# TravisDai/DLRM-FlexFlow

Measured on AMD Instinct MI355X. Metric: samples/sec DLRM (MLPerf-like) at 1/2/4/8 MI355X; SOAP speedup vs pure DP, higher is better.
Workload: dtype fp32; 1 GPU; global_batch=8192, seq_len=1, parallelism=dp1, tables_rows=187767399, embedding_dim=128, interaction=dot, hip_graph=True, backend=none, process_world=1, fp32_gemm=bf16x3-split-big+native-f32-mfma, gemm_tuned_entries=21, gemm_staging=lds-dma

## Files before the change

csrc/kernels/embedding.hip:

```cpp
#include "common.h"

#include <algorithm>
#include <cstdlib>
#include <cstring>
#include <vector>

namespace {

constexpr int MAXT = 32;
constexpr int TINY_ROWS = 16;

struct TabDesc {
  const float* W;
  const void* idx;
  void* act;
  long ld;
  long lo;
  int rows, D, bag;
  float scale;
};

FM_DEVICE long local_row(long r, long lo, int rows, bool& ok) {
  const long l = r - lo;
  ok = (unsigned long)l < (unsigned long)rows;
  return ok ? l : 0;
}
struct TabSet {
  TabDesc t[MAXT];
  int n;
};

template <bool I64>
FM_DEVICE long ldi(const void* p, long i) {
  if constexpr (I64) return (long)reinterpret_cast<const long long*>(p)[i];
  else return (long)reinterpret_cast<const int*>(p)[i];
}

template <typename OutT, bool I64>
__global__ void __launch_bounds__(256) fm_emb_fwd_multi(TabSet s, long B, int su) {
  const TabDesc& d = s.t[blockIdx.y];
  const int D4 = d.D >> 2;
  const int lpr = D4 < 64 ? D4 : 64;
  const int rpi = 256 / lpr;
  const int sub = threadIdx.x / lpr, lc = threadIdx.x - sub * lpr;
  if (sub >= rpi) return;
  const long bstride = (long)gridDim.x * rpi;
  if (su && d.bag == 1 && D4 <= 64) {
    constexpr int SU = 4;
    const int c = lc * 4;
    for (long b0 = (long)blockIdx.x * rpi + sub; b0 < B; b0 += SU * bstride) {
      long r[SU];
      bool ok[SU];
#pragma unroll
      for (int u = 0; u < SU; ++u) r[u] = local_row(ldi<I64>(d.idx, min(b0 + u * bstride, B - 1)), d.lo, d.rows, ok[u]);
      f32x4_t v[SU];
#pragma unroll
      for (int u = 0; u < SU; ++u) v[u] = *reinterpret_cast<const f32x4_t*>(d.W + r[u] * d.D + c);
#pragma unroll
      for (int u = 0; u < SU; ++u) {
        const long b = b0 + u * bstride;
        if (b >= B) break;
        f32x4_t acc = ok[u] ? v[u] * d.scale : f32x4_t{0.f, 0.f, 0.f, 0.f};
        OutT* o = reinterpret_cast<OutT*>(d.act) + b * d.ld + c;
        if constexpr (sizeof(OutT) == 4) {
          *reinterpret_cast<f32x4_t*>(o) = acc;
        } else {
          bf16x4_t w;
          w[0] = (short)f2bf(acc[0]); w[1] = (short)f2bf(acc[1]); w[2] = (short)f2bf(acc[2]); w[3] = (short)f2bf(acc[3]);
          *reinterpret_cast<bf16x4_t*>(o) = w;
        }
      }
    }
    return;
  }
  for (long b = (long)blockIdx.x * rpi + sub; b < B; b += bstride) {
    for (int c4 = lc; c4 < D4; c4 += lpr) {
      const int c = c4 * 4;
      f32x4_t acc = {0.f, 0.f, 0.f, 0.f};
      int j = 0;
      for (; j + 8 <= d.bag; j += 8) {
        long r[8];
        bool ok[8];
#pragma unroll
        for (int u = 0; u < 8; ++u) r[u] = local_row(ldi<I64>(d.idx, b * d.bag + j + u), d.lo, d.rows, ok[u]);
        f32x4_t v[8];
#pragma unroll
        for (int u = 0; u < 8; ++u) v[u] = *reinterpret_cast<const f32x4_t*>(d.W + r[u] * d.D + c);
#pragma unroll
        for (int u = 0; u < 8; ++u)
          if (ok[u]) acc += v[u];
      }
      for (; j < d.bag; ++j) {
        bool ok;
        const long r = local_row(ldi<I64>(d.idx, b * d.bag + j), d.lo, d.rows, ok);
        const f32x4_t v = *reinterpret_cast<const f32x4_t*>(d.W + r * d.D + c);
        if (ok) acc += v;
      }
      acc *= d.scale;
      OutT* o = reinterpret_cast<OutT*>(d.act) + b * d.ld + c;
      if constexpr (sizeof(OutT) == 4) {
        *reinterpret_cast<f32x4_t*>(o) = acc;
      } else {
        bf16x4_t v;
        v[0] = (short)f2bf(acc[0]); v[1] = (short)f2bf(acc[1]); v[2] = (short)f2bf(acc[2]); v[3] = (short)f2bf(acc[3]);
        *reinterpret_cast<bf16x4_t*>(o) = v;
      }
    }
  }
}

template <typename OutT, bool I64>
__global__ void __launch_bounds__(256) fm_emb_fwd_split(TabSet s, long B, int sp) {
  __shared__ f32x4_t part[256];
  const TabDesc& d = s.t[blockIdx.y];
  const int lpr = d.D >> 2;
  const int rpi = 256 / lpr;
  const int spb = rpi / sp;
  const int sub = threadIdx.x / lpr, lc = threadIdx.x - sub * lpr;
  const bool live = sub < spb * sp;
  const int si = sub / sp, k = sub - si * sp;
  const long b = (long)blockIdx.x * spb + si;
  f32x4_t acc = {0.f, 0.f, 0.f, 0.f};
  if (live && b < B) {
    const int c = lc * 4;
    int j = k;
    for (; j + 3 * sp < d.bag; j += 4 * sp) {
      long r[4];
      bool ok[4];
#pragma unroll
      for (int u = 0; u < 4; ++u) r[u] = local_row(ldi<I64>(d.idx, b * d.bag + j + u * sp), d.lo, d.rows, ok[u]);
      f32x4_t v[4];
#pragma unroll
      for (int u = 0; u < 4; ++u) v[u] = *reinterpret_cast<const f32x4_t*>(d.W + r[u] * d.D + c);
#pragma unroll
      for (int u = 0; u < 4; ++u)
        if (ok[u]) acc += v[u];
    }
    for (; j < d.bag; j += sp) {
      bool ok;
      const long r = local_row(ldi<I64>(d.idx, b * d.bag + j), d.lo, d.rows, ok);
      const f32x4_t v = *reinterpret_cast<const f32x4_t*>(d.W + r * d.D + c);
      if (ok) acc += v;
    }
  }
  part[threadIdx.x] = acc;
  __syncthreads();
  if (!live || k != 0 || b >= B) return;
  for (int q = 1; q < sp; ++q) acc += part[threadIdx.x + q * lpr];
  acc *= d.scale;
  OutT* o = reinterpret_cast<OutT*>(d.act) + b * d.ld + lc * 4;
  if constexpr (sizeof(OutT) == 4) {
    *reinterpret_cast<f32x4_t*>(o) = acc;
  } else {
    bf16x4_t v;
    v[0] = (short)f2bf(acc[0]); v[1] = (short)f2bf(acc[1]); v[2] = (short)f2bf(acc[2]); v[3] = (short)f2bf(acc[3]);
    *reinterpret_cast<bf16x4_t*>(o) = v;
  }
}

template <typename OutT, bool I64>
__global__ void __launch_bounds__(256) fm_emb_fwd_multi_scalar(TabSet s, long B) {
  const TabDesc& d = s.t[blockIdx.y];
  const int lpr = d.D < 256 ? d.D : 256;
  const int rpi = 256 / lpr;
  const int sub = threadIdx.x / lpr, lc = threadIdx.x - sub * lpr;
  if (sub >= rpi) return;
  for (long b = (long)blockIdx.x * rpi + sub; b < B; b += (long)gridDim.x * rpi)
    for (int c = lc; c < d.D; c += lpr) {
      float acc = 0.f;
      for (int j = 0; j < d.bag; ++j) {
        bool ok;
        const long r = local_row(ldi<I64>(d.idx, b * d.bag + j), d.lo, d.rows, ok);
        const float v = d.W[r * d.D + c];
        if (ok) acc += v;
      }
      st<OutT>(reinterpret_cast<OutT*>(d.act) + b * d.ld + c, acc * d.scale);
    }
}

template <typename GT, bool I64>
__global__ void __launch_bounds__(256) fm_emb_bwd_atomic_multi(TabSet s, const float* __restrict__ lr, long B) {
  const TabDesc& d = s.t[blockIdx.y];
  const float mul = (lr ? -lr[0] : 1.f) * d.scale;
  const int lpr = d.D < 256 ? d.D : 256;
  const int rpi = 256 / lpr;
  const int sub = threadIdx.x / lpr, lc = threadIdx.x - sub * lpr;
  if (sub >= rpi) return;
  float* W = const_cast<float*>(d.W);
  const GT* dy = reinterpret_cast<const GT*>(d.act);
  for (long b = (long)blockIdx.x * rpi + sub; b < B; b += (long)gridDim.x * rpi) {
    bool ok0;
    const long r0 = local_row(ldi<I64>(d.idx, b * d.bag), d.lo, d.rows, ok0);
    for (int c = lc; c < d.D; c += lpr) {
      const float g = ld<GT>(dy + b * d.ld + c) * mul;
      if (ok0) atomicAdd(W + r0 * d.D + c, g);
      for (int j = 1; j < d.bag; ++j) {
        bool ok;
        const long r = local_row(ldi<I64>(d.idx, b * d.bag + j), d.lo, d.rows, ok);
        if (ok) atomicAdd(W + r * d.D + c, g);
      }
    }
  }
}

template <typename GT, bool I64>
__global__ void __launch_bounds__(256) fm_emb_bwd_tiny_multi(TabSet s, const float* __restrict__ lr, long B, int chunk) {
  constexpr int S = 16;
  extern __shared__ __attribute__((aligned(16))) char smem[];
  float* red = reinterpret_cast<float*>(smem);
  const TabDesc& d = s.t[blockIdx.y];
  const long b0 = (long)blockIdx.x * chunk;
  if (b0 >= B) return;
  const long b1 = min(B, b0 + chunk);
  const int wave = threadIdx.x >> 6, lane = threadIdx.x & 63;
  const int n = d.rows * d.D;
  float* mine = red + wave * n;
  for (int i = lane; i < n; i += 64) mine[i] = 0.f;
  const GT* dy = reinterpret_cast<const GT*>(d.act);
  for (long bw = b0 + (long)wave * S; bw < b1; bw += 4L * S) {
    for (int c0 = 0; c0 < d.D; c0 += 128) {
      const int ca = c0 + lane, cb = c0 + 64 + lane;
      const int sa = min(ca, d.D - 1), sb = min(cb, d.D - 1);
      long r[S];
      bool rok[S];
      float ga[S], gb[S];
#pragma unroll
      for (int u = 0; u < S; ++u) {
        const long bu = min(bw + u, b1 - 1);
        r[u] = local_row(ldi<I64>(d.idx, bu * d.bag), d.lo, d.rows, rok[u]);
        ga[u] = ld<GT>(dy + bu * d.ld + sa);
        gb[u] = ld<GT>(dy + bu * d.ld + sb);
      }
#pragma unroll
      for (int u = 0; u < S; ++u) {
        if (bw + u >= b1) break;
        float* p = mine + r[u] * d.D;
        if (rok[u] && ca < d.D) p[ca] += ga[u];
        if (rok[u] && cb < d.D) p[cb] += gb[u];
        for (int j = 1; j < d.bag; ++j) {
          bool ok;
          float* q = mine + local_row(ldi<I64>(d.idx, (bw + u) * d.bag + j), d.lo, d.rows, ok) * d.D;
          if (ok && ca < d.D) q[ca] += ga[u];
          if (ok && cb < d.D) q[cb] += gb[u];
        }
      }
    }
  }
  __syncthreads();
  const float mul = (lr ? -lr[0] : 1.f) * d.scale;
  float* W = const_cast<float*>(d.W);
  for (int i = threadIdx.x; i < n; i += 256) {
    const float v = red[i] + red[n + i] + red[2 * n + i] + red[3 * n + i];
    if (v != 0.f) atomicAdd(W + i, v * mul);
  }
}

template <bool I64>
void launch_fwd(const TabSet& s, int m, bool vec, bool out_bf16, long B, int D0, hipStream_t st) {
  const int rpi = std::max(1, 256 / std::min(64, std::max(1, D0 / 4)));
  int minbag = 1 << 30, maxD = 0, minD = 1 << 30;
  for (int i = 0; i < m; ++i) {
    minbag = std::min(minbag, s.t[i].bag);
    maxD = std::max(maxD, s.t[i].D);
    minD = std::min(minD, s.t[i].D);
  }
  if (vec && maxD == minD && maxD <= 256 && minbag >= 16 && (B + rpi - 1) / rpi * m < 1024) {
    int sp = 1;
    while (sp * 2 <= rpi && sp * 2 <= minbag / 4 && (B * sp * 2 + rpi - 1) / rpi * m <= 2048) sp *= 2;
    if (sp > 1) {
      const int spb = rpi / sp;
      dim3 grid((unsigned)((B + spb - 1) / spb), m);
      if (out_bf16) hipLaunchKernelGGL((fm_emb_fwd_split<unsigned short, I64>), grid, dim3(256), 0, st, s, B, sp);
      else hipLaunchKernelGGL((fm_emb_fwd_split<float, I64>), grid, dim3(256), 0, st, s, B, sp);
      return;
    }
  }
  dim3 grid((unsigned)std::max<long>(1, std::min<long>((B + rpi - 1) / rpi, 256L)), m);
  const int su = 1;
  if (vec) {
    if (out_bf16) hipLaunchKernelGGL((fm_emb_fwd_multi<unsigned short, I64>), grid, dim3(256), 0, st, s, B, su);
    else hipLaunchKernelGGL((fm_emb_fwd_multi<float, I64>), grid, dim3(256), 0, st, s, B, su);
  } else {
    if (out_bf16) hipLaunchKernelGGL((fm_emb_fwd_multi_scalar<unsigned short, I64>), grid, dim3(256), 0, st, s, B);
    else hipLaunchKernelGGL((fm_emb_fwd_multi_scalar<float, I64>), grid, dim3(256), 0, st, s, B);
  }
}

struct ClaimDesc {
  float* W;
  const void* idx;
  const void* dy;
  long ld;
  long lo;
  int rows, D, bag;
  float scale;
  int* owner;
  int* dups;
  int* ndup;
};
struct ClaimSet {
  ClaimDesc t[MAXT];
  int n;
};

template <bool I64>
__global__ void __launch_bounds__(256) fm_emb_claim_multi(ClaimSet s, long B) {
  const ClaimDesc& d = s.t[blockIdx.y];
  const long n = B * d.bag;
  for (long e = blockIdx.x * 256L + threadIdx.x; e < n; e += (long)gridDim.x * 256) {
    bool ok;
    const long r = local_row(ldi<I64>(d.idx, e), d.lo, d.rows, ok);
    if (!ok) continue;
    const int prev = atomicCAS(d.owner + r, -1, (int)e);
    if (prev != -1) d.dups[atomicAdd(d.ndup, 1)] = (int)e;
  }
}

template <typename GT, bool I64>
__global__ void __launch_bounds__(256) fm_emb_dup_multi(ClaimSet s, const float* __restrict__ lr) {
  const ClaimDesc& d = s.t[blockIdx.y];
  const int nd = *d.ndup;
  const float mul = -lr[0] * d.scale;
  const int wave = threadIdx.x >> 6, lane = threadIdx.x & 63;
  const GT* dy = reinterpret_cast<const GT*>(d.dy);
  for (long k = blockIdx.x * 4L + wave; k < nd; k += (long)gridDim.x * 4) {
    const long e = d.dups[k];
    const long b = e / d.bag, r = ldi<I64>(d.idx, e) - d.lo;
    for (int c = lane; c < d.D; c += 64) atomicAdd(d.W + r * d.D + c, ld<GT>(dy + b * d.ld + c) * mul);
  }
}

template <typename GT, bool I64>
__global__ void __launch_bounds__(256) fm_emb_owner_multi(ClaimSet s, const float* __restrict__ lr, long B) {
  const ClaimDesc& d = s.t[blockIdx.y];
  const float mul = -lr[0] * d.scale;
  const int D4 = d.D >> 2;
  const int lpr = D4 < 64 ? D4 : 64;
  const int rpi = 256 / lpr;
  const int sub = threadIdx.x / lpr, lc = threadIdx.x - sub * lpr;
  const long n = B * d.bag;
  const GT* dy = reinterpret_cast<const GT*>(d.dy);
  if (sub < rpi) {
    for (long e = (long)blockIdx.x * rpi + sub; e < n; e += (long)gridDim.x * rpi) {
      bool ok;
      const long r = local_row(ldi<I64>(d.idx, e), d.lo, d.rows, ok);
      if (!ok || d.owner[r] != (int)e) continue;
      const long b = e / d.bag;
      for (int c4 = lc; c4 < D4; c4 += lpr) {
        const int c = c4 * 4;
        f32x4_t* wp = reinterpret_cast<f32x4_t*>(d.W + r * d.D + c);
        f32x4_t w = *wp;
        if constexpr (sizeof(GT) == 2) {
          const bf16x4_t g = *reinterpret_cast<const bf16x4_t*>(dy + b * d.ld + c);
#pragma unroll
          for (int j = 0; j < 4; ++j) w[j] += mul * bf2f((unsigned short)g[j]);
        } else {
          const f32x4_t g = *reinterpret_cast<const f32x4_t*>(dy + b * d.ld + c);
          w += mul * g;
        }
        *wp = w;
      }
      if (lc == 0) d.owner[r] = -1;
    }
  }
  if (blockIdx.x == 0 && threadIdx.x == 0) *d.ndup = 0;
}

template <bool I64>
__global__ void __launch_bounds__(256) fm_emb_count_multi(ClaimSet s, long B) {
  const ClaimDesc& d = s.t[blockIdx.y];
  const long n = B * d.bag;
  for (long e = blockIdx.x * 256L + threadIdx.x; e < n; e += (long)gridDim.x * 256) {
    bool ok;
    const long r = local_row(ldi<I64>(d.idx, e), d.lo, d.rows, ok);
    int own = 0;
    if (ok) own = atomicAdd(d.owner + r, 1) == -1;
    d.dups[e] = own;
  }
}

template <typename GT, bool I64>
__global__ void __launch_bounds__(256) fm_emb_update_multi(ClaimSet s, const float* __restrict__ lr, long B) {
  const ClaimDesc& d = s.t[blockIdx.y];
  const float mul = -lr[0] * d.scale;
  const int D4 = d.D >> 2;
  const int lpr = D4 < 64 ? D4 : 64;
  const int rpi = 256 / lpr;
  const int sub = threadIdx.x / lpr, lc = threadIdx.x - sub * lpr;
  const long n = B * d.bag;
  const GT* dy = reinterpret_cast<const GT*>(d.dy);
  if (sub >= rpi) return;
  for (long e = (long)blockIdx.x * rpi + sub; e < n; e += (long)gridDim.x * rpi) {
    bool ok;
    const long r = local_row(ldi<I64>(d.idx, e), d.lo, d.rows, ok);
    if (!ok) continue;
    const int c = __hip_atomic_load(d.owner + r, __ATOMIC_RELAXED, __HIP_MEMORY_SCOPE_AGENT);
    const int own = d.dups[e];
    const long b = e / d.bag;
    const GT* g = dy + b * d.ld;
    float* wr = d.W + r * d.D;
    if (c == 0) {
      for (int c4 = lc; c4 < D4; c4 += lpr) {
        const int col = c4 * 4;
        f32x4_t* wp = reinterpret_cast<f32x4_t*>(wr + col);
        f32x4_t w = *wp;
        if constexpr (sizeof(GT) == 2) {
          const bf16x4_t gv = *reinterpret_cast<const bf16x4_t*>(g + col);
#pragma unroll
          for (int j = 0; j < 4; ++j) w[j] += mul * bf2f((unsigned short)gv[j]);
        } else {
          w += mul * *reinterpret_cast<const f32x4_t*>(g + col);
        }
        *wp = w;
      }
    } else {
      for (int col = lc; col < d.D; col += lpr) atomicAdd(wr + col, mul * ld<GT>(g + col));
    }
    if (lc == 0 && (c == 0 || own)) __hip_atomic_store(d.owner + r, -1, __ATOMIC_RELAXED, __HIP_MEMORY_SCOPE_AGENT);
  }
}

template <bool I64>
void launch_count(const ClaimSet& s, int m, bool dy_bf16, const float* lr, long B, int maxbag, int minD4,
                  hipStream_t st) {
  const long n = B * maxbag;
  dim3 gc((unsigned)std::max<long>(1, std::min<long>((n + 255) / 256, 1024)), m);
  hipLaunchKernelGGL((fm_emb_count_multi<I64>), gc, dim3(256), 0, st, s, B);
  const int rpi = 256 / std::min(64, std::max(1, minD4));
  dim3 gu((unsigned)std::max<long>(1, std::min<long>((n + rpi - 1) / rpi, 2048)), m);
  if (dy_bf16) hipLaunchKernelGGL((fm_emb_update_multi<unsigned short, I64>), gu, dim3(256), 0, st, s, lr, B);
  else hipLaunchKernelGGL((fm_emb_update_multi<float, I64>), gu, dim3(256), 0, st, s, lr, B);
}

long emb_bwd_cap(long want) { return want; }

template <bool I64>
void launch_claim(const ClaimSet& s, int m, bool dy_bf16, const float* lr, long B, int maxbag, int minD4,
                  hipStream_t st) {
  const long n = B * maxbag;
  dim3 gc((unsigned)std::max<long>(1, emb_bwd_cap(std::min<long>((n + 255) / 256, 1024))), m);
  hipLaunchKernelGGL((fm_emb_claim_multi<I64>), gc, dim3(256), 0, st, s, B);
  dim3 gd((unsigned)std::max<long>(1, emb_bwd_cap(std::min<long>((n + 3) / 4, 1024))), m);
  if (dy_bf16) hipLaunchKernelGGL((fm_emb_dup_multi<unsigned short, I64>), gd, dim3(256), 0, st, s, lr);
  else hipLaunchKernelGGL((fm_emb_dup_multi<float, I64>), gd, dim3(256), 0, st, s, lr);
  const int rpi = 256 / std::min(64, std::max(1, minD4));
  dim3 go((unsigned)std::max<long>(1, emb_bwd_cap(std::min<long>((n + rpi - 1) / rpi, 2048))), m);
  if (dy_bf16) hipLaunchKernelGGL((fm_emb_owner_multi<unsigned short, I64>), go, dim3(256), 0, st, s, lr, B);
  else hipLaunchKernelGGL((fm_emb_owner_multi<float, I64>), go, dim3(256), 0, st, s, lr, B);
}

template <bool I64>
void launch_bwd(const TabSet& s, int m, bool tiny, bool dy_bf16, const float* lr, long B, int maxD, hipStream_t st) {
  if (tiny) {
    size_t lds = 0;
    for (int i = 0; i < m; ++i) lds = std::max(lds, (size_t)s.t[i].rows * s.t[i].D * 4 * 4);
    static bool attr = false;
    if (!attr) {
      (void)hipFuncSetAttribute((const void*)fm_emb_bwd_tiny_multi<unsigned short, I64>,
                                hipFuncAttributeMaxDynamicSharedMemorySize, 160 << 10);
      (void)hipFuncSetAttribute((const void*)fm_emb_bwd_tiny_multi<float, I64>,
                                hipFuncAttributeMaxDynamicSharedMemorySize, 160 << 10);
      attr = true;
    }
    const int chunk = B <= 16384 ? 64 : B <= 32768 ? 128 : 256;
    dim3 grid((unsigned)((B + chunk - 1) / chunk), m);
    if (dy_bf16) hipLaunchKernelGGL((fm_emb_bwd_tiny_multi<unsigned short, I64>), grid, dim3(256), lds, st, s, lr, B, chunk);
    else hipLaunchKernelGGL((fm_emb_bwd_tiny_multi<float, I64>), grid, dim3(256), lds, st, s, lr, B, chunk);
  } else {
    const int rpi = std::max(1, 256 / std::min(256, maxD));
    dim3 grid((unsigned)std::max<long>(1, emb_bwd_cap(std::min<long>((B + rpi - 1) / rpi, 2048))), m);
    if (dy_bf16) hipLaunchKernelGGL((fm_emb_bwd_atomic_multi<unsigned short, I64>), grid, dim3(256), 0, st, s, lr, B);
    else hipLaunchKernelGGL((fm_emb_bwd_atomic_multi<float, I64>), grid, dim3(256), 0, st, s, lr, B);
  }
}

struct SdpDesc {
  const void* idx;
  const void* dy;
  long ld;
  long lo;
  int rows, D, bag;
  float scale;
  int* slot;
  int* cid;
  int* ids;
  float* g;
  int* count;
};
struct SdpSet {
  SdpDesc t[MAXT];
  int n;
};

template <bool I64>
__global__ void __launch_bounds__(256) fm_sdp_claim(SdpSet s, long B) {
  const SdpDesc& d = s.t[blockIdx.y];
  const long n = B * d.bag;
  for (long e = blockIdx.x * 256L + threadIdx.x; e < n; e += (long)gridDim.x * 256) {
    bool ok;
    const long r = local_row(ldi<I64>(d.idx, e), d.lo, d.rows, ok);
    if (ok) atomicCAS(d.slot + r, -1, (int)e);
  }
}

template <typename GT, bool I64>
__global__ void __launch_bounds__(256) fm_sdp_assign(SdpSet s, long B) {
  const SdpDesc& d = s.t[blockIdx.y];
  const int wave = threadIdx.x >> 6, lane = threadIdx.x & 63;
  const long n = B * d.bag;
  const GT* dy = reinterpret_cast<const GT*>(d.dy);
  for (long e = blockIdx.x * 4L + wave; e < n; e += (long)gridDim.x * 4) {
    bool ok;
    const long r = local_row(ldi<I64>(d.idx, e), d.lo, d.rows, ok);
    if (!ok || d.slot[r] != (int)e) continue;
    int u = 0;
    if (lane == 0) u = atomicAdd(d.count, 1);
    u = __shfl(u, 0, 64);
    const long b = e / d.bag;
    float* gu = d.g + (long)u * d.D;
    for (int c = lane; c < d.D; c += 64) gu[c] = ld<GT>(dy + b * d.ld + c) * d.scale;
    if (lane == 0) {
      d.ids[u] = (int)r;
      d.cid[e] = u;
    }
  }
}

template <typename GT, bool I64>
__global__ void __launch_bounds__(256) fm_sdp_dups(SdpSet s, long B) {
  const SdpDesc& d = s.t[blockIdx.y];
  const int wave = threadIdx.x >> 6, lane = threadIdx.x & 63;
  const long n = B * d.bag;
  const GT* dy = reinterpret_cast<const GT*>(d.dy);
  for (long e = blockIdx.x * 4L + wave; e < n; e += (long)gridDim.x * 4) {
    bool ok;
    const long r = local_row(ldi<I64>(d.idx, e), d.lo, d.rows, ok);
    if (!ok) continue;
    const int own = d.slot[r];
    if (own == (int)e) continue;
    const long b = e / d.bag;
    float* gu = d.g + (long)d.cid[own] * d.D;
    for (int c = lane; c < d.D; c += 64) atomicAdd(gu + c, ld<GT>(dy + b * d.ld + c) * d.scale);
  }
}

struct SdpApply {
  float* W;
  const int* ids;
  const float* g;
  const int* count;
  int D;
  int* slot;
  int* own_count;
};
struct SdpApplySet {
  SdpApply t[MAXT];
  int n;
};

__global__ void __launch_bounds__(256) fm_sdp_apply(SdpApplySet s, const float* __restrict__ lr, int nmax) {
  const SdpApply& d = s.t[blockIdx.y];
  const int wave = threadIdx.x >> 6, lane = threadIdx.x & 63;
  const int cnt = min(*d.count, nmax);
  const float mlr = -lr[0];
  for (long u = blockIdx.x * 4L + wave; u < cnt; u += (long)gridDim.x * 4) {
    const long r = d.ids[u];
    float* w = d.W + r * d.D;
    const float* gu = d.g + u * d.D;
    for (int c = lane; c < d.D; c += 64) w[c] += mlr * gu[c];
    if (d.slot && lane == 0) d.slot[r] = -1;
  }
}

struct CountSet {
  int* c[MAXT] = {};
};
__global__ void fm_emb_zero_counts(CountSet s) {
  if (threadIdx.x < MAXT && s.c[threadIdx.x]) *s.c[threadIdx.x] = 0;
}

struct AdaDesc {
  float* W;
  float* H;
  const int* ids;
  const float* g;
  int* count;
  int* slot;
  int D, nmax, vec;
};
struct AdaSet {
  AdaDesc t[MAXT];
  int n;
};

__global__ void __launch_bounds__(256) fm_emb_adagrad_apply_multi(AdaSet s, const float* __restrict__ lr_p, float eps) {
  const AdaDesc& d = s.t[blockIdx.y];
  const long cnt = min(*d.count, d.nmax);
  if (cnt <= 0) return;
  const float lr = lr_p[0];
  if (d.vec) {
    const int D4 = d.D >> 2;
    const int lpr = D4 < 64 ? D4 : 64;
    const int rpi = 256 / lpr;
    const int sub = threadIdx.x / lpr, lc = threadIdx.x - sub * lpr;
    if (sub >= rpi) return;
    const long stride = (long)gridDim.x * rpi;
    for (long u0 = (long)blockIdx.x * rpi + sub; u0 < cnt; u0 += 2 * stride) {
      const bool live1 = u0 + stride < cnt;
      const long u1 = live1 ? u0 + stride : cnt - 1;
      const long r0 = d.ids[u0], r1 = d.ids[u1];
      for (int c4 = lc; c4 < D4; c4 += lpr) {
        const int c = c4 * 4;
        f32x4_t* hp0 = reinterpret_cast<f32x4_t*>(d.H + r0 * d.D + c);
        f32x4_t* wp0 = reinterpret_cast<f32x4_t*>(d.W + r0 * d.D + c);
        f32x4_t* hp1 = reinterpret_cast<f32x4_t*>(d.H + r1 * d.D + c);
        f32x4_t* wp1 = reinterpret_cast<f32x4_t*>(d.W + r1 * d.D + c);
        const f32x4_t g0 = *reinterpret_cast<const f32x4_t*>(d.g + u0 * d.D + c);
        const f32x4_t g1 = *reinterpret_cast<const f32x4_t*>(d.g + u1 * d.D + c);
        f32x4_t h0 = *hp0, h1 = *hp1, w0 = *wp0, w1 = *wp1;
        h0 += g0 * g0;
        h1 += g1 * g1;
#pragma unroll
        for (int j = 0; j < 4; ++j) {
          w0[j] -= lr * g0[j] / (sqrtf(h0[j]) + eps);
          w1[j] -= lr * g1[j] / (sqrtf(h1[j]) + eps);
        }
        *hp0 = h0;
        *wp0 = w0;
        if (live1) {
          *hp1 = h1;
          *wp1 = w1;
        }
      }
      if (lc == 0) {
        d.slot[r0] = -1;
        if (live1) d.slot[r1] = -1;
      }
    }
  } else {
    const int wave = threadIdx.x >> 6, lane = threadIdx.x & 63;
    for (long u = blockIdx.x * 4L + wave; u < cnt; u += (long)gridDim.x * 4) {
      const long r = d.ids[u];
      float* h = d.H + r * d.D;
      float* w = d.W + r * d.D;
      const float* gu = d.g + u * d.D;
      for (int c = lane; c < d.D; c += 64) {
        const float g = gu[c];
        const float hc = h[c] + g * g;
        h[c] = hc;
        w[c] -= lr * g / (sqrtf(hc) + eps);
      }
      if (lane == 0) d.slot[r] = -1;
    }
  }
}

__device__ inline float sumsq4(const f32x4_t v) { return v[0] * v[0] + v[1] * v[1] + v[2] * v[2] + v[3] * v[3]; }

__global__ void __launch_bounds__(256) fm_emb_rowwise_apply_multi(AdaSet s, const float* __restrict__ lr_p, float eps) {
  const AdaDesc& d = s.t[blockIdx.y];
  const long cnt = min(*d.count, d.nmax);
  if (cnt <= 0) return;
  const float lr = lr_p[0];
  const float invD = 1.0f / (float)d.D;
  if (d.vec) {
    const int D4 = d.D >> 2;
    const int act = D4 < 64 ? D4 : 64;
    int G = 1;
    while (G < act) G <<= 1;
    const int rpi = 256 / G;
    const int sub = threadIdx.x / G, lc = threadIdx.x & (G - 1);
    const bool col = lc < act;
    const int c0 = (col ? lc : 0) * 4;
    for (long base = (long)blockIdx.x * rpi; base < cnt; base += (long)gridDim.x * rpi) {
      const bool live = base + sub < cnt;
      const long u = live ? base + sub : cnt - 1;
      const long r = d.ids[u];
      const f32x4_t gv = *reinterpret_cast<const f32x4_t*>(d.g + u * d.D + c0);
      const f32x4_t w = *reinterpret_cast<const f32x4_t*>(d.W + r * d.D + c0);
      const float hv = d.H[r];
      float ss = col ? sumsq4(gv) : 0.0f;
      for (int c4 = lc + 64; c4 < D4; c4 += 64)
        ss += sumsq4(*reinterpret_cast<const f32x4_t*>(d.g + u * d.D + c4 * 4));
      for (int off = G >> 1; off > 0; off >>= 1) ss += __shfl_xor(ss, off, 64);
      const float hn = hv + ss * invD;
      const float mul = lr / (sqrtf(hn) + eps);
      if (live && col) {
        *reinterpret_cast<f32x4_t*>(d.W + r * d.D + c0) = w - mul * gv;
        for (int c4 = lc + 64; c4 < D4; c4 += 64) {
          f32x4_t* wp = reinterpret_cast<f32x4_t*>(d.W + r * d.D + c4 * 4);
          *wp = *wp - mul * *reinterpret_cast<const f32x4_t*>(d.g + u * d.D + c4 * 4);
        }
      }
      if (live && lc == 0) {
        d.H[r] = hn;
        d.slot[r] = -1;
      }
    }
  } else {
    const int wave = threadIdx.x >> 6, lane = threadIdx.x & 63;
    for (long u = blockIdx.x * 4L + wave; u < cnt; u += (long)gridDim.x * 4) {
      const long r = d.ids[u];
      float* w = d.W + r * d.D;
      const float* gu = d.g + u * d.D;
      float ss = 0.0f;
      for (int c = lane; c < d.D; c += 64) ss += gu[c] * gu[c];
      for (int off = 32; off > 0; off >>= 1) ss += __shfl_xor(ss, off, 64);
      const float hn = d.H[r] + ss * invD;
      const float mul = lr / (sqrtf(hn) + eps);
      for (int c = lane; c < d.D; c += 64) w[c] -= mul * gu[c];
      if (lane == 0) {
        d.H[r] = hn;
        d.slot[r] = -1;
      }
    }
  }
}

struct RwMerge {
  const int* ids;
  const float* g;
  const int* count;
  int* slot;
  int* mids;
  float* mg;
  int* mcount;
  int rows, D, nmax, mcap, vec;
};
struct RwMergeSet {
  RwMerge t[MAXT];
  int n;
};
struct RwRelease {
  const int* ids;
  int* count;
  int* slot;
  int rows, nmax;
};
struct RwReleaseSet {
  RwRelease t[MAXT];
  int n;
};

__global__ void __launch_bounds__(256) fm_sdp_rowwise_release(RwReleaseSet s) {
  const RwRelease& d = s.t[blockIdx.y];
  const long cnt = min(*d.count, d.nmax);
  for (long u = blockIdx.x * 256L + threadIdx.x; u < cnt; u += (long)gridDim.x * 256) {
    const int r = d.ids[u];
    if ((unsigned)r < (unsigned)d.rows) d.slot[r] = -1;
  }
}

__global__ void __launch_bounds__(256) fm_sdp_rowwise_merge(RwMergeSet s) {
  const RwMerge& d = s.t[blockIdx.y];
  const int wave = threadIdx.x >> 6, lane = threadIdx.x & 63;
  const long cnt = min(*d.count, d.nmax);
  for (long u = blockIdx.x * 4L + wave; u < cnt; u += (long)gridDim.x * 4) {
    const int r = d.ids[u];
    if ((unsigned)r >= (unsigned)d.rows) continue;
    int m = 0;
    if (lane == 0) {
      m = d.slot[r];
      if (m < 0) {
        m = atomicAdd(d.mcount, 1);
        if (m < d.mcap) {
          d.slot[r] = m;
          d.mids[m] = r;
        }
        m = ~m;
      }
    }
    m = __shfl(m, 0, 64);
    const bool first = m < 0;
    if (first) m = ~m;
    if (m >= d.mcap) continue;
    const float* gu = d.g + u * d.D;
    float* mo = d.mg + (long)m * d.D;
    if (d.vec) {
      for (int c4 = lane; c4 < (d.D >> 2); c4 += 64) {
        const f32x4_t v = *reinterpret_cast<const f32x4_t*>(gu + c4 * 4);
        f32x4_t* mp = reinterpret_cast<f32x4_t*>(mo + c4 * 4);
        *mp = first ? v : *mp + v;
      }
    } else {
      for (int c = lane; c < d.D; c += 64) mo[c] = first ? gu[c] : mo[c] + gu[c];
    }
  }
}

}

extern "C" void fm_embedding_fwd_multi(int n, const float* const* W, const void* const* idx, const int* idx64,
                                       void* const* out, const long* ldo, const long* lo, const int* rows, const int* D,
                                       const int* bag, const float* scale, int out_bf16, long B, hipStream_t st) {
  if (B <= 0) return;
  for (int wide = 0; wide < 2; ++wide) {
    std::vector<int> sel;
    for (int k = 0; k < n; ++k)
      if ((idx64[k] != 0) == (wide != 0)) sel.push_back(k);
    for (size_t base = 0; base < sel.size(); base += MAXT) {
      TabSet s;
      int m = (int)std::min<size_t>(MAXT, sel.size() - base);
      bool vec = true;
      for (int i = 0; i < m; ++i) {
        int k = sel[base + i];
        s.t[i] = TabDesc{W[k], idx[k], out[k], ldo[k], lo ? lo[k] : 0, rows[k], D[k], bag[k], scale[k]};
        vec = vec && (D[k] % 4 == 0) && (ldo[k] % 4 == 0) && D[k] <= 256;
      }
      s.n = m;
      if (wide) launch_fwd<true>(s, m, vec, out_bf16, B, D[sel[base]], st);
      else launch_fwd<false>(s, m, vec, out_bf16, B, D[sel[base]], st);
    }
  }
}

static int g_emb_count = 0;
extern "C" void fm_embedding_set_bwd_mode(int count) { g_emb_count = count ? 1 : 0; }

extern "C" void fm_embedding_bwd_multi(int n, float* const* W, const void* const* idx, const int* idx64,
                                       const void* const* dy, const long* ldg, const long* lo, const int* rows, const int* D,
                                       const int* bag, const float* scale, int dy_bf16, const float* lr, long B,
                                       int* const* owner, int* const* dups, int* const* ndup, hipStream_t st) {
  if (B <= 0) return;
  const bool count_mode = g_emb_count == 1;
  auto claimable = [&](int k) {
    return lr != nullptr && owner != nullptr && owner[k] != nullptr && D[k] % 4 == 0 && ldg[k] % 4 == 0 &&
           D[k] <= 256;
  };
  for (int wide = 0; wide < 2; ++wide) {
    std::vector<int> sel;
    for (int k = 0; k < n; ++k)
      if (claimable(k) && (idx64[k] != 0) == (wide != 0)) sel.push_back(k);
    for (size_t base = 0; base < sel.size(); base += MAXT) {
      ClaimSet s;
      int m = (int)std::min<size_t>(MAXT, sel.size() - base);
      int maxbag = 1, minD4 = 64;
      for (int i = 0; i < m; ++i) {
        int k = sel[base + i];
        s.t[i] = ClaimDesc{W[k], idx[k], dy[k], ldg[k], lo ? lo[k] : 0, rows[k], D[k], bag[k], scale[k], owner[k], dups[k],
                           ndup[k]};
        maxbag = std::max(maxbag, bag[k]);
        minD4 = std::min(minD4, D[k] / 4);
      }
      s.n = m;
      if (count_mode) {
        if (wide) launch_count<true>(s, m, dy_bf16, lr, B, maxbag, minD4, st);
        else launch_count<false>(s, m, dy_bf16, lr, B, maxbag, minD4, st);
      } else if (wide) {
        launch_claim<true>(s, m, dy_bf16, lr, B, maxbag, minD4, st);
      } else {
        launch_claim<false>(s, m, dy_bf16, lr, B, maxbag, minD4, st);
      }
    }
  }
  auto kind_of = [&](int k) {
    constexpr int tiny_rows = 64;
    if (rows[k] <= tiny_rows && (long)rows[k] * D[k] * 16 <= (160L << 10) && D[k] <= 256 &&
        B * (long)bag[k] >= 16L * rows[k])
      return 0;
    return 2;
  };
  for (int pass = 0; pass < 4; ++pass) {
    const int kind = (pass >> 1) * 2;
    const bool tiny = kind == 0, wide = pass & 1;
    std::vector<int> sel;
    for (int k = 0; k < n; ++k) {
      if (claimable(k)) continue;
      if (kind_of(k) == kind && (idx64[k] != 0) == wide) sel.push_back(k);
    }
    for (size_t base = 0; base < sel.size(); base += MAXT) {
      TabSet s;
      int m = (int)std::min<size_t>(MAXT, sel.size() - base);
      int maxD = 1;
      for (int i = 0; i < m; ++i) {
        int k = sel[base + i];
        s.t[i] = TabDesc{W[k], idx[k], const_cast<void*>(dy[k]), ldg[k], lo ? lo[k] : 0, rows[k], D[k], bag[k], scale[k]};
        maxD = std::max(maxD, D[k]);
      }
      s.n = m;
      if (wide) {
        launch_bwd<true>(s, m, tiny, dy_bf16, lr, B, maxD, st);
      } else {
        launch_bwd<false>(s, m, tiny, dy_bf16, lr, B, maxD, st);
      }
    }
  }
}

extern "C" void fm_embedding_fwd(const void* idx, int idx64, const float* W, void* out, int out_bf16, long B, int bag,
                                 int rows, int D, long ldo, float scale, hipStream_t s) {
  fm_embedding_fwd_multi(1, &W, &idx, &idx64, &out, &ldo, nullptr, &rows, &D, &bag, &scale, out_bf16, B, s);
}

extern "C" void fm_embedding_bwd(const void* idx, int idx64, const void* dy, int dy_bf16, float* W, const float* lr,
                                 long B, int bag, int rows, int D, long ldg, float scale, hipStream_t s) {
  fm_embedding_bwd_multi(1, &W, &idx, &idx64, &dy, &ldg, nullptr, &rows, &D, &bag, &scale, dy_bf16, lr, B, nullptr,
                         nullptr, nullptr, s);
}

template <typename GT, bool I64>
static void launch_coalesce(const SdpSet& s, dim3 gc, dim3 gw, long B, hipStream_t st) {
  hipLaunchKernelGGL((fm_sdp_claim<I64>), gc, dim3(256), 0, st, s, B);
  hipLaunchKernelGGL((fm_sdp_assign<GT, I64>), gw, dim3(256), 0, st, s, B);
  hipLaunchKernelGGL((fm_sdp_dups<GT, I64>), gw, dim3(256), 0, st, s, B);
}

extern "C" void fm_sdp_coalesce(int n, const void* const* idx, const int* idx64, const void* const* dy, const long* ldg,
                                const long* lo, const int* rows, const int* D, const int* bag, const float* scale,
                                int dy_bf16, long B, int* const* slot, int* const* cid, int* const* ids, float* const* g,
                                int* const* count, hipStream_t st) {
  if (B <= 0 || n <= 0) return;
  static constexpr decltype(&launch_coalesce<float, false>) launch[2][2] = {
      {launch_coalesce<float, false>, launch_coalesce<float, true>},
      {launch_coalesce<unsigned short, false>, launch_coalesce<unsigned short, true>}};
  for (int wide = 0; wide < 2; ++wide) {
    std::vector<int> sel;
    for (int k = 0; k < n; ++k)
      if ((idx64[k] != 0) == (wide != 0)) sel.push_back(k);
    for (size_t base = 0; base < sel.size(); base += MAXT) {
      SdpSet s;
      const int m = (int)std::min<size_t>(MAXT, sel.size() - base);
      int maxbag = 1;
      for (int i = 0; i < m; ++i) {
        const int k = sel[base + i];
        s.t[i] = SdpDesc{idx[k], dy[k], ldg[k], lo ? lo[k] : 0, rows[k], D[k], bag[k], scale[k], slot[k], cid[k], ids[k],
                         g[k], count[k]};
        maxbag = std::max(maxbag, bag[k]);
      }
      s.n = m;
      const long ne = B * maxbag;
      dim3 gc((unsigned)std::max<long>(1, std::min<long>((ne + 255) / 256, 1024)), m);
      dim3 gw((unsigned)std::max<long>(1, std::min<long>((ne + 3) / 4, 2048)), m);
      launch[dy_bf16 != 0][wide](s, gc, gw, B, st);
    }
  }
}

extern "C" void fm_sdp_apply_segments(int n, int segs, int own_seg, float* const* W, const int* D, const int* const* seg_ids,
                                      const float* const* seg_g, const int* const* seg_count, int* const* slot,
                                      int* const* own_count, const int* nmax, const float* lr, hipStream_t st) {
  if (n <= 0) return;
  for (size_t base = 0; base < (size_t)n; base += MAXT) {
    const int m = (int)std::min<size_t>(MAXT, n - base);
    int nm = 1;
    for (int i = 0; i < m; ++i) nm = std::max(nm, nmax[base + i]);
    dim3 grid((unsigned)std::max(1, std::min((nm + 3) / 4, 2048)), m);
    CountSet zero;
    for (int sg = 0; sg < segs; ++sg) {
      SdpApplySet s;
      for (int i = 0; i < m; ++i) {
        const int k = (int)base + i;
        const bool own = sg == own_seg;
        s.t[i] = SdpApply{W[k], seg_ids[sg * n + k], seg_g[sg * n + k], seg_count[sg * n + k], D[k], own ? slot[k] : nullptr,
                          own ? own_count[k] : nullptr};
        if (own) zero.c[i] = own_count[k];
      }
      s.n = m;
      hipLaunchKernelGGL(fm_sdp_apply, grid, dim3(256), 0, st, s, lr, nm);
    }
    if (own_seg >= 0 && own_seg < segs) hipLaunchKernelGGL(fm_emb_zero_counts, dim3(1), dim3(64), 0, st, zero);
  }
}

static void launch_adagrad_apply(void (*kernel)(AdaSet, const float*, float), bool h_vec, int n, float* const* W,
                                 float* const* H, const int* D, const int* const* ids, const float* const* g,
                                 int* const* count, int* const* slot, const int* nmax, const float* lr, float eps,
                                 hipStream_t st) {
  if (n <= 0) return;
  for (size_t base = 0; base < (size_t)n; base += MAXT) {
    const int m = (int)std::min<size_t>(MAXT, n - base);
    AdaSet s;
    CountSet zero;
    int nm = 1;
    for (int i = 0; i < m; ++i) {
      const int k = (int)base + i;
      const uintptr_t a = ((uintptr_t)W[k]) | ((uintptr_t)g[k]) | (h_vec ? (uintptr_t)H[k] : 0);
      const bool vec = D[k] % 4 == 0 && (a & 15) == 0;
      s.t[i] = AdaDesc{W[k], H[k], ids[k], g[k], count[k], slot[k], D[k], nmax[k], vec ? 1 : 0};
      zero.c[i] = count[k];
      nm = std::max(nm, nmax[k]);
    }
    s.n = m;
    dim3 grid((unsigned)std::max(1, std::min((nm + 7) / 8, 2048)), m);
    hipLaunchKernelGGL(kernel, grid, dim3(256), 0, st, s, lr, eps);
    hipLaunchKernelGGL(fm_emb_zero_counts, dim3(1), dim3(64), 0, st, zero);
  }
}

extern "C" void fm_emb_adagrad_apply(int n, float* const* W, float* const* H, const int* D, const int* const* ids,
                                     const float* const* g, int* const* count, int* const* slot, const int* nmax,
                                     const float* lr, float eps, hipStream_t st) {
  launch_adagrad_apply(fm_emb_adagrad_apply_multi, true, n, W, H, D, ids, g, count, slot, nmax, lr, eps, st);
}

extern "C" void fm_emb_rowwise_adagrad_apply(int n, float* const* W, float* const* h, const int* D,
                                             const int* const* ids, const float* const* g, int* const* count,
                                             int* const* slot, const int* nmax, const float* lr, float eps,
                                             hipStream_t st) {
  launch_adagrad_apply(fm_emb_rowwise_apply_multi, false, n, W, h, D, ids, g, count, slot, nmax, lr, eps, st);
}

extern "C" void fm_sdp_rowwise_merge_segments(int n, int segs, const int* rows, const int* D, const int* const* seg_ids,
                                              const float* const* seg_g, const int* const* seg_count,
                                              const int* const* own_ids, int* const* own_count, int* const* slot,
                                              int* const* mids, float* const* mg, int* const* mcount, const int* nmax,
                                              const int* mcap, hipStream_t st) {
  if (n <= 0) return;
  for (size_t base = 0; base < (size_t)n; base += MAXT) {
    const int m = (int)std::min<size_t>(MAXT, n - base);
    int nm = 1;
    RwReleaseSet rs;
    CountSet zero;
    for (int i = 0; i < m; ++i) {
      const int k = (int)base + i;
      rs.t[i] = RwRelease{own_ids[k], own_count[k], slot[k], rows[k], nmax[k]};
      zero.c[i] = own_count[k];
      nm = std::max(nm, nmax[k]);
    }
    rs.n = m;
    hipLaunchKernelGGL(fm_sdp_rowwise_release, dim3((unsigned)std::max(1, std::min((nm + 255) / 256, 1024)), m), dim3(256),
                       0, st, rs);
    hipLaunchKernelGGL(fm_emb_zero_counts, dim3(1), dim3(64), 0, st, zero);
    dim3 grid((unsigned)std::max(1, std::min((nm + 3) / 4, 2048)), m);
    for (int sg = 0; sg < segs; ++sg) {
      RwMergeSet s;
      for (int i = 0; i < m; ++i) {
        const int k = (int)base + i;
        const float* gs = seg_g[sg * n + k];
        const bool vec = D[k] % 4 == 0 && ((((uintptr_t)gs) | ((uintptr_t)mg[k])) & 15) == 0;
        s.t[i] = RwMerge{seg_ids[sg * n + k], gs, seg_count[sg * n + k], slot[k], mids[k], mg[k], mcount[k],
                         rows[k], D[k], nmax[k], mcap[k], vec ? 1 : 0};
      }
      s.n = m;
      hipLaunchKernelGGL(fm_sdp_rowwise_merge, grid, dim3(256), 0, st, s);
    }
  }
}
```

Measured before the change: 7.162 million samples/s.

## Use MFMA one-hot accumulation for tiny-table backward and fuse claim/dup kernels

Replaces the LDS-reduction backward for small embedding tables with a kernel that builds one-hot row counts and accumulates gradients via 16x16x4 f32 MFMA, with triple-buffered prefetch of indices and gradients and a per-wave staging flush to atomics. Separately merges the claim and duplicate-scatter kernels: lost CAS claims are handled in-wave via ballot, which removes the dups list, the global ndup counter and one kernel launch. The aim is to cut LDS traffic, shared-memory footprint and launch count in the embedding backward. It adds MFMA-specific code paths, new vector-alignment eligibility conditions and more complex indexing.

```diff
diff --git a/csrc/kernels/embedding.hip b/csrc/kernels/embedding.hip
--- a/csrc/kernels/embedding.hip
+++ b/csrc/kernels/embedding.hip
@@ -3,12 +3,12 @@
 #include <algorithm>
 #include <cstdlib>
 #include <cstring>
+#include <type_traits>
 #include <vector>
 
 namespace {
 
 constexpr int MAXT = 32;
-constexpr int TINY_ROWS = 16;
 
 struct TabDesc {
   const float* W;
@@ -203,55 +203,108 @@
   }
 }
 
+constexpr int ONEHOT_ROWS = 64;
+constexpr int ONEHOT_SUB = 256;
+struct OneHotSet {
+  TabDesc t[MAXT];
+  int ustart[MAXT + 1];
+  int n;
+};
+inline __host__ __device__ int onehot_wr(int rows) { return rows > 32 ? 4 : rows > 16 ? 2 : 1; }
+
+FM_DEVICE void onehot_wave_sync() {
+  __builtin_amdgcn_fence(__ATOMIC_RELEASE, "workgroup");
+  __builtin_amdgcn_wave_barrier();
+  __builtin_amdgcn_fence(__ATOMIC_ACQUIRE, "workgroup");
+}
+
 template <typename GT, bool I64>
-__global__ void __launch_bounds__(256) fm_emb_bwd_tiny_multi(TabSet s, const float* __restrict__ lr, long B, int chunk) {
-  constexpr int S = 16;
-  extern __shared__ __attribute__((aligned(16))) char smem[];
-  float* red = reinterpret_cast<float*>(smem);
-  const TabDesc& d = s.t[blockIdx.y];
-  const long b0 = (long)blockIdx.x * chunk;
-  if (b0 >= B) return;
-  const long b1 = min(B, b0 + chunk);
-  const int wave = threadIdx.x >> 6, lane = threadIdx.x & 63;
-  const int n = d.rows * d.D;
-  float* mine = red + wave * n;
-  for (int i = lane; i < n; i += 64) mine[i] = 0.f;
+__global__ void __launch_bounds__(256, 2) fm_emb_bwd_onehot_multi(OneHotSet s, const float* __restrict__ lr, long B) {
+  __shared__ __attribute__((aligned(16))) float stage_all[4][16 * 64];
+  constexpr int U = 8;
+  constexpr int S = 4 * U;
+  using IdxT = typename std::conditional<I64, long long, int>::type;
+  using RawT = typename std::conditional<sizeof(GT) == 2, bf16x4_t, f32x4_t>::type;
+  int ti = 0;
+  while (ti + 1 < s.n && (int)blockIdx.x >= s.ustart[ti + 1]) ++ti;
+  const TabDesc& d = s.t[ti];
+  const int ub = (int)blockIdx.x - s.ustart[ti];
+  const int nsl = (d.D + 63) >> 6;
+  const int cb = ub / nsl, c0 = (ub - cb * nsl) * 64;
+  const int wave = threadIdx.x >> 6, lane = threadIdx.x & 63, k = lane >> 4, r16 = lane & 15;
+  const int wr = onehot_wr(d.rows);
+  const int tile = wave & (wr - 1);
+  const long bs = ((long)cb * (4 / wr) + wave / wr) * ONEHOT_SUB;
+  if (bs >= B || tile * 16 >= d.rows) return;
+  const long be = min(B, bs + ONEHOT_SUB);
+  const int cl = min(c0 + 4 * r16, d.D - 4);
   const GT* dy = reinterpret_cast<const GT*>(d.act);
-  for (long bw = b0 + (long)wave * S; bw < b1; bw += 4L * S) {
-    for (int c0 = 0; c0 < d.D; c0 += 128) {
-      const int ca = c0 + lane, cb = c0 + 64 + lane;
-      const int sa = min(ca, d.D - 1), sb = min(cb, d.D - 1);
-      long r[S];
-      bool rok[S];
-      float ga[S], gb[S];
-#pragma unroll
-      for (int u = 0; u < S; ++u) {
-        const long bu = min(bw + u, b1 - 1);
-        r[u] = local_row(ldi<I64>(d.idx, bu * d.bag), d.lo, d.rows, rok[u]);
-        ga[u] = ld<GT>(dy + bu * d.ld + sa);
-        gb[u] = ld<GT>(dy + bu * d.ld + sb);
-      }
-#pragma unroll
-      for (int u = 0; u < S; ++u) {
-        if (bw + u >= b1) break;
-        float* p = mine + r[u] * d.D;
-        if (rok[u] && ca < d.D) p[ca] += ga[u];
-        if (rok[u] && cb < d.D) p[cb] += gb[u];
-        for (int j = 1; j < d.bag; ++j) {
-          bool ok;
-          float* q = mine + local_row(ldi<I64>(d.idx, (bw + u) * d.bag + j), d.lo, d.rows, ok) * d.D;
-          if (ok && ca < d.D) q[ca] += ga[u];
-          if (ok && cb < d.D) q[cb] += gb[u];
-        }
-      }
-    }
-  }
-  __syncthreads();
+  const IdxT* idx = reinterpret_cast<const IdxT*>(d.idx);
+  const int rid = tile * 16 + r16;
+  f32x4_t acc[4];
+#pragma unroll
+  for (int v = 0; v < 4; ++v) acc[v] = f32x4_t{0.f, 0.f, 0.f, 0.f};
+  auto fetch = [&](long bb, IdxT& ix, RawT (&g)[U]) {
+    const long base = min(bb, be - 1);
+    const int last = (int)min((long)(S - 1), be - 1 - base);
+    ix = idx[(base + min(lane, last)) * d.bag];
+    const GT* p = dy + base * d.ld;
+#pragma unroll
+    for (int u = 0; u < U; ++u)
+      g[u] = *reinterpret_cast<const RawT*>(p + ((unsigned)min(4 * u + k, last) * (unsigned)d.ld + (unsigned)cl));
+  };
+  auto row_of = [&](long r, bool live) {
+    bool ok;
+    const long l = local_row(r, d.lo, d.rows, ok);
+    return (ok && live) ? (int)l : -1;
+  };
+  auto sum = [&](long bb, IdxT ix, const RawT (&g)[U]) {
+    const int mine = row_of((long)ix, lane < S && bb + lane < be);
+#pragma unroll
+    for (int u = 0; u < U; ++u) {
+      float cnt = __shfl(mine, 4 * u + k, 64) == rid ? 1.f : 0.f;
+      if (d.bag > 1) {
+        const long b = bb + 4 * u + k;
+        const long bc = min(b, be - 1);
+        for (int j = 1; j < d.bag; ++j) cnt += row_of((long)idx[bc * d.bag + j], b < be) == rid ? 1.f : 0.f;
+      }
+      f32x4_t gv;
+      if constexpr (sizeof(GT) == 2) {
+        gv = f32x4_t{bf2f((unsigned short)g[u][0]), bf2f((unsigned short)g[u][1]), bf2f((unsigned short)g[u][2]),
+                     bf2f((unsigned short)g[u][3])};
+      } else {
+        gv = g[u];
+      }
+#pragma unroll
+      for (int v = 0; v < 4; ++v) acc[v] = __builtin_amdgcn_mfma_f32_16x16x4f32(cnt, gv[v], acc[v], 0, 0, 0);
+    }
+  };
+  IdxT ia, ib, ic;
+  RawT ga[U], gb[U], gc[U];
+  fetch(bs, ia, ga);
+  fetch(bs + S, ib, gb);
+  for (long bb = bs; bb < be; bb += 3 * S) {
+    fetch(bb + 2 * S, ic, gc);
+    sum(bb, ia, ga);
+    fetch(bb + 3 * S, ia, ga);
+    if (bb + S < be) sum(bb + S, ib, gb);
+    fetch(bb + 4 * S, ib, gb);
+    if (bb + 2 * S < be) sum(bb + 2 * S, ic, gc);
+  }
+  float* stage = stage_all[wave];
+#pragma unroll
+  for (int i = 0; i < 4; ++i)
+    *reinterpret_cast<f32x4_t*>(stage + (4 * k + i) * 64 + 4 * r16) = f32x4_t{acc[0][i], acc[1][i], acc[2][i], acc[3][i]};
+  onehot_wave_sync();
   const float mul = (lr ? -lr[0] : 1.f) * d.scale;
   float* W = const_cast<float*>(d.W);
-  for (int i = threadIdx.x; i < n; i += 256) {
-    const float v = red[i] + red[n + i] + red[2 * n + i] + red[3 * n + i];
-    if (v != 0.f) atomicAdd(W + i, v * mul);
+  if (c0 + lane < d.D) {
+#pragma unroll
+    for (int r = 0; r < 16; ++r) {
+      const float v = stage[r * 64 + lane];
+      const int row = tile * 16 + r;
+      if (row < d.rows && v != 0.f) atomicAdd(W + (long)row * d.D + c0 + lane, v * mul);
+    }
   }
 }
 
@@ -303,30 +356,43 @@
   int n;
 };
 
-template <bool I64>
-__global__ void __launch_bounds__(256) fm_emb_claim_multi(ClaimSet s, long B) {
+constexpr int CLAIM_EPW = 16;
+
+template <typename GT, bool I64>
+__global__ void __launch_bounds__(256) fm_emb_claim_multi(ClaimSet s, const float* __restrict__ lr, long B) {
+  constexpr int G = 8;
   const ClaimDesc& d = s.t[blockIdx.y];
   const long n = B * d.bag;
-  for (long e = blockIdx.x * 256L + threadIdx.x; e < n; e += (long)gridDim.x * 256) {
+  const float mul = -lr[0] * d.scale;
+  const int lane = threadIdx.x & 63;
+  const GT* dy = reinterpret_cast<const GT*>(d.dy);
+  for (long e0 = (blockIdx.x * 4L + (threadIdx.x >> 6)) * CLAIM_EPW; e0 < n; e0 += (long)gridDim.x * 4 * CLAIM_EPW) {
+    const long e = e0 + lane;
     bool ok;
-    const long r = local_row(ldi<I64>(d.idx, e), d.lo, d.rows, ok);
-    if (!ok) continue;
-    const int prev = atomicCAS(d.owner + r, -1, (int)e);
-    if (prev != -1) d.dups[atomicAdd(d.ndup, 1)] = (int)e;
-  }
-}
-
-template <typename GT, bool I64>
-__global__ void __launch_bounds__(256) fm_emb_dup_multi(ClaimSet s, const float* __restrict__ lr) {
-  const ClaimDesc& d = s.t[blockIdx.y];
-  const int nd = *d.ndup;
-  const float mul = -lr[0] * d.scale;
-  const int wave = threadIdx.x >> 6, lane = threadIdx.x & 63;
-  const GT* dy = reinterpret_cast<const GT*>(d.dy);
-  for (long k = blockIdx.x * 4L + wave; k < nd; k += (long)gridDim.x * 4) {
-    const long e = d.dups[k];
-    const long b = e / d.bag, r = ldi<I64>(d.idx, e) - d.lo;
-    for (int c = lane; c < d.D; c += 64) atomicAdd(d.W + r * d.D + c, ld<GT>(dy + b * d.ld + c) * mul);
+    const int r = (int)local_row(ldi<I64>(d.idx, min(e, n - 1)), d.lo, d.rows, ok);
+    bool lost = false;
+    if (ok && lane < CLAIM_EPW && e < n) lost = atomicCAS(d.owner + r, -1, (int)e) != -1;
+    unsigned long long m = __ballot(lost);
+    while (m) {
+      long gb[G], wb[G];
+      bool live[G];
+#pragma unroll
+      for (int q = 0; q < G; ++q) {
+        live[q] = m != 0;
+        const int src = live[q] ? __ffsll(m) - 1 : 0;
+        m &= m - 1;
+        gb[q] = (e0 + src) / d.bag * d.ld;
+        wb[q] = (long)__shfl(r, src, 64) * d.D;
+      }
+      for (int c = lane; c < d.D; c += 64) {
+        float g[G];
+#pragma unroll
+        for (int q = 0; q < G; ++q) g[q] = ld<GT>(dy + gb[q] + c);
+#pragma unroll
+        for (int q = 0; q < G; ++q)
+          if (live[q]) atomicAdd(d.W + wb[q] + c, g[q] * mul);
+      }
+    }
   }
 }
 
@@ -363,7 +429,6 @@
       if (lc == 0) d.owner[r] = -1;
     }
   }
-  if (blockIdx.x == 0 && threadIdx.x == 0) *d.ndup = 0;
 }
 
 template <bool I64>
@@ -438,11 +503,10 @@
 void launch_claim(const ClaimSet& s, int m, bool dy_bf16, const float* lr, long B, int maxbag, int minD4,
                   hipStream_t st) {
   const long n = B * maxbag;
-  dim3 gc((unsigned)std::max<long>(1, emb_bwd_cap(std::min<long>((n + 255) / 256, 1024))), m);
-  hipLaunchKernelGGL((fm_emb_claim_multi<I64>), gc, dim3(256), 0, st, s, B);
-  dim3 gd((unsigned)std::max<long>(1, emb_bwd_cap(std::min<long>((n + 3) / 4, 1024))), m);
-  if (dy_bf16) hipLaunchKernelGGL((fm_emb_dup_multi<unsigned short, I64>), gd, dim3(256), 0, st, s, lr);
-  else hipLaunchKernelGGL((fm_emb_dup_multi<float, I64>), gd, dim3(256), 0, st, s, lr);
+  const long epb = 4L * CLAIM_EPW;
+  dim3 gc((unsigned)std::max<long>(1, emb_bwd_cap(std::min<long>((n + epb - 1) / epb, 1024))), m);
+  if (dy_bf16) hipLaunchKernelGGL((fm_emb_claim_multi<unsigned short, I64>), gc, dim3(256), 0, st, s, lr, B);
+  else hipLaunchKernelGGL((fm_emb_claim_multi<float, I64>), gc, dim3(256), 0, st, s, lr, B);
   const int rpi = 256 / std::min(64, std::max(1, minD4));
   dim3 go((unsigned)std::max<long>(1, emb_bwd_cap(std::min<long>((n + rpi - 1) / rpi, 2048))), m);
   if (dy_bf16) hipLaunchKernelGGL((fm_emb_owner_multi<unsigned short, I64>), go, dim3(256), 0, st, s, lr, B);
@@ -450,22 +514,19 @@
 }
 
 template <bool I64>
-void launch_bwd(const TabSet& s, int m, bool tiny, bool dy_bf16, const float* lr, long B, int maxD, hipStream_t st) {
-  if (tiny) {
-    size_t lds = 0;
-    for (int i = 0; i < m; ++i) lds = std::max(lds, (size_t)s.t[i].rows * s.t[i].D * 4 * 4);
-    static bool attr = false;
-    if (!attr) {
-      (void)hipFuncSetAttribute((const void*)fm_emb_bwd_tiny_multi<unsigned short, I64>,
-                                hipFuncAttributeMaxDynamicSharedMemorySize, 160 << 10);
-      (void)hipFuncSetAttribute((const void*)fm_emb_bwd_tiny_multi<float, I64>,
-                                hipFuncAttributeMaxDynamicSharedMemorySize, 160 << 10);
-      attr = true;
-    }
-    const int chunk = B <= 16384 ? 64 : B <= 32768 ? 128 : 256;
-    dim3 grid((unsigned)((B + chunk - 1) / chunk), m);
-    if (dy_bf16) hipLaunchKernelGGL((fm_emb_bwd_tiny_multi<unsigned short, I64>), grid, dim3(256), lds, st, s, lr, B, chunk);
-    else hipLaunchKernelGGL((fm_emb_bwd_tiny_multi<float, I64>), grid, dim3(256), lds, st, s, lr, B, chunk);
+void launch_bwd(const TabSet& s, int m, bool onehot, bool dy_bf16, const float* lr, long B, int maxD, hipStream_t st) {
+  if (onehot) {
+    OneHotSet o;
+    o.n = m;
+    o.ustart[0] = 0;
+    for (int i = 0; i < m; ++i) {
+      o.t[i] = s.t[i];
+      const long per_block = (long)ONEHOT_SUB * (4 / onehot_wr(s.t[i].rows));
+      o.ustart[i + 1] = o.ustart[i] + (int)((B + per_block - 1) / per_block) * ((s.t[i].D + 63) / 64);
+    }
+    dim3 grid((unsigned)o.ustart[m]);
+    if (dy_bf16) hipLaunchKernelGGL((fm_emb_bwd_onehot_multi<unsigned short, I64>), grid, dim3(256), 0, st, o, lr, B);
+    else hipLaunchKernelGGL((fm_emb_bwd_onehot_multi<float, I64>), grid, dim3(256), 0, st, o, lr, B);
   } else {
     const int rpi = std::max(1, 256 / std::min(256, maxD));
     dim3 grid((unsigned)std::max<long>(1, emb_bwd_cap(std::min<long>((B + rpi - 1) / rpi, 2048))), m);
@@ -854,15 +915,14 @@
     }
   }
   auto kind_of = [&](int k) {
-    constexpr int tiny_rows = 64;
-    if (rows[k] <= tiny_rows && (long)rows[k] * D[k] * 16 <= (160L << 10) && D[k] <= 256 &&
-        B * (long)bag[k] >= 16L * rows[k])
-      return 0;
+    const bool vec = D[k] >= 4 && D[k] % 4 == 0 && ldg[k] % 4 == 0 && ldg[k] < (1L << 24) &&
+                     ((uintptr_t)dy[k] & (dy_bf16 ? 7 : 15)) == 0;
+    if (rows[k] >= 1 && rows[k] <= ONEHOT_ROWS && vec && D[k] <= 256) return 0;
     return 2;
   };
   for (int pass = 0; pass < 4; ++pass) {
     const int kind = (pass >> 1) * 2;
-    const bool tiny = kind == 0, wide = pass & 1;
+    const bool onehot = kind == 0, wide = pass & 1;
     std::vector<int> sel;
     for (int k = 0; k < n; ++k) {
       if (claimable(k)) continue;
@@ -879,9 +939,9 @@
       }
       s.n = m;
       if (wide) {
-        launch_bwd<true>(s, m, tiny, dy_bf16, lr, B, maxD, st);
+        launch_bwd<true>(s, m, onehot, dy_bf16, lr, B, maxD, st);
       } else {
-        launch_bwd<false>(s, m, tiny, dy_bf16, lr, B, maxD, st);
+        launch_bwd<false>(s, m, onehot, dy_bf16, lr, B, maxD, st);
       }
     }
   }
```

New measurement: 7.190 million samples/s (median of 6 runs). No clear change (+0.4%).
